# yjhuangcd/FI-ODE

Hardware: AMD Instinct MI355X
Metric: CIFAR-10 train-step images/sec (B=128, h_sample=256) at 1/2/4/8 MI355X (higher is better)
Workload: dtype f32; 1 GPU; hipGraph replay: BASELINE configs[1]: train step of README.md:27 at epoch 20 with train_ode (rk4, step_size 0.1, t_max=1: 10 steps / 40 train-mode f-evals, backprop through the stages; loss_ode portion 0.2) + the Lyapunov loss (B=128, h_sample_size=256 -> 204 uniform + 52 correct-cone rows/image), KWLarge-Cayley backbone + Adam; global_batch=128, h_sample_size=256, rows_per_rank=32768, parallelism=dp1

## Files before the change

### fi-ode_amd/csrc/odetrain.hip

```cpp
#include <type_traits>
#include "common.h"
#include "tile.h"
#include "tile16.h"
#include "tile4.h"
#include "wgrad.h"
#include "dopri5.h"
#include "../../include/fiode.h"

namespace {
using namespace fiode_tile;
using namespace fiode_t16;
using namespace fiode_t4;
using namespace fiode_dp;


constexpr int OT_XRING = 4;
constexpr int FIODE_OT_KW_PRE = 256;

struct OTArgs {
  int prio;
  int B, E, niters;
  int nslots;
  int kw_lazy;
  int kw_pre;
// ... 317 lines not shown
    store_row10(a.ftw + r * C, ft);
    store_row10(a.nomw + r * C, nominal);
    store_row10(a.loww + r * C, lower);
    store_row10(a.vw + r * C, k);
    a.muw[r] = mu;
  }
  if (blockIdx.x == 0 && threadIdx.x == 0) a.stats[2] = K;
#ifdef OT_PROFILE
  if (blockIdx.x == 0 && threadIdx.x == 0 && e < 96) a.prof[16 + e] = (unsigned long long)K;
#endif
  if (threadIdx.x == 0) sh.Kprev = K;
  if (end_barrier) __syncthreads();
  OT_MARK(4);
}

__global__ __launch_bounds__(256) void k_ot_fwd4(OTArgs a) {
  fiode_wave_prio(a.prio & 1);
  extern __shared__ __attribute__((aligned(16))) float smem[];
  OtShared4& sh = *reinterpret_cast<OtShared4*>(smem);
  if (threadIdx.x == 0) {
    sh.Kprev = a.d.max_iter - 1;
    sh.dead = 0;
  }
  const int lane = threadIdx.x & 63, j = lane & 3;
  const int p = __builtin_amdgcn_readfirstlane(threadIdx.x >> 6);
  const int b = blockIdx.x * TR4 + j;
  const bool valid = b < a.B;
  const int bb = valid ? b : a.B - 1;
  T4W w;
  load_t4w(a.Q1, a.Q2, a.Q3, a.b2, a.b3, p, lane, w);
  for (int t = threadIdx.x; t < TR4 * M; t += blockDim.x) {
    const int rb = blockIdx.x * TR4 + t / M, i = t % M;
    if (rb < a.B) {
      float s = 0.f;
#pragma unroll
      for (int c = 0; c < FIODE_X; ++c) s = __fmaf_rn(a.Qx[i * FIODE_X + c], a.x_feat[(size_t)rb * FIODE_X + c], s);
      a.u[(size_t)rb * M + i] = (s + a.bx[i]) + a.b1[i];
    }
  }
  __syncthreads();
  const f32x4 uacc = *reinterpret_cast<const f32x4*>(a.u + (size_t)bb * M + 32 * p + 4 * ((lane >> 2) & 7));
  const uint32_t* kwp = a.kw;
  auto fetch = [&](int e, uint32_t& w1, uint32_t& w2) {
    if (a.dropout_mode == FIODE_DROPOUT_OFF) {
      w1 = w2 = 0xFFFFFFFFu;
      return;
    }
    w1 = kwp[(((size_t)e * 2 + 0) * a.B + bb) * 4 + p];
    w2 = kwp[(((size_t)e * 2 + 1) * a.B + bb) * 4 + p];
  };
  uint32_t kc1, kc2, kn1 = 0u, kn2 = 0u;
  fetch(0, kc1, kc2);
  float y[C], k1[C], k2[C], k3[C], k4[C], hin[C];
  load_row10(a.h0 + (size_t)bb * C, y);
  const float third = 1.0f / 3.0f;
  const int eN = 4 * (a.niters - 1);
  for (int it = 0; it + 1 < a.niters; ++it) {
    float ta, dt;
    step_times(a, it, ta, dt);
    const int e0 = 4 * it;
#define OT4_STAGE(E_, H_, K_)                                                            \
    {                                                                                    \
      if ((E_) + 1 < eN) fetch((E_) + 1, kn1, kn2);                                      \
      ot_eval4(a, w, sh, (E_), p, b, valid, lane, j, uacc, kc1, kc2, H_, K_, false);    \
      kc1 = kn1;                                                                         \
      kc2 = kn2;                                                                         \
    }
    OT4_STAGE(e0, y, k1)
// ... 10 lines not shown
#pragma unroll
    for (int i = 0; i < C; ++i) {
      const float dy = (((k1[i] + 3.0f * (k2[i] + k3[i])) + k4[i]) * dt) * 0.125f;
      y[i] = y[i] + dy;
    }
  }
  if (sh.dead) {
#pragma unroll
    for (int i = 0; i < C; ++i) y[i] = __builtin_nanf("");
  }
  if (p == 0 && valid && lane < TR4) store_row10(a.y_out + (size_t)b * C, y);
  if (blockIdx.x == 0 && threadIdx.x == 0) {
    a.stats[0] = 4 * (a.niters - 1);
    a.stats[1] = a.niters - 1;
  }
}

struct OtBwdShared {
  float gpart[2][4][64][4];
  float gax[8][64][4];
};

struct VjpIn {
  float h[C], ft[C], v[C], mu;
  f32x4 a2[2];
  f32x4 a1[2];
};

__device__ __forceinline__ void load_vjp_in(const OTArgs& a, int p, int e, int b, bool valid, int q, VjpIn& in) {
  const int bb = valid ? b : a.B - 1;
// ... 340 lines not shown
  if (blk4 < 4) *reinterpret_cast<f32x4*>(&sh.gpart[buf][p][lane][0]) = f32x4{gh[0], gh[1], gh[2], gh[3]};
  OT_MARK(13);
  __syncthreads();
  OT_MARK(14);
#pragma unroll
  for (int i = 0; i < C; ++i) {
    const int ln = 4 * (i >> 2) + j, rg = i & 3;
    const float ghm = ((sh.gpart[buf][0][ln][rg] + sh.gpart[buf][1][ln][rg]) + sh.gpart[buf][2][ln][rg]) +
                      sh.gpart[buf][3][ln][rg];
    gy_out[i] = ghm + ghb[i];
  }
  OT_MARK(15);
}

template <bool SN>
__global__ __launch_bounds__(256) void k_ot_bwd4(OTArgs a) {
  fiode_wave_prio(a.prio & 2);
  extern __shared__ __attribute__((aligned(16))) float smem[];
  OtBwdShared4& sh = *reinterpret_cast<OtBwdShared4*>(smem);
  const int lane = threadIdx.x & 63, j = lane & 3;
  const int p = __builtin_amdgcn_readfirstlane(threadIdx.x >> 6);
  VjpW4 wv;
  {
    const int bq = lane >> 2, i = lane & 3;
    const int u = 32 * p + 4 * (bq & 7) + i;
#pragma unroll
    for (int s = 0; s < 5; ++s) wv.q3t[s] = a.Q3[(s + 5 * (bq >> 3)) * M + u];
#pragma unroll
    for (int s = 0; s < 64; ++s) wv.q2t[s] = a.Q2[(size_t)(s + 64 * (bq >> 3)) * M + u];
    const int c = 4 * (bq & 3) + i;
#pragma unroll
    for (int s = 0; s < 8; ++s) wv.q1t[s] = c < C ? a.Q1[(32 * p + 8 * (bq >> 2) + s) * C + c] : 0.f;
  }
  const int b = blockIdx.x * TR4 + j;
  const bool valid = b < a.B;
  float gy[C];
  if (valid) load_row10(a.g_y + (size_t)b * C, gy);
  else
#pragma unroll
    for (int i = 0; i < C; ++i) gy[i] = 0.f;
  const float third = 1.0f / 3.0f;
  int buf = 0;
  VjpIn4 cur, nxt;
  VjpRow crw;
  load_vjp_in4(a, p, a.E - 1, b, valid, lane, cur);
#define OT_VJP4(E_, G_)                                                                 \
  load_vjp_in4(a, p, (E_) - 1, b, valid, lane, nxt);                                    \
  vjp_row_math<SN>(a, cur, crw);                                                        \
  ot_vjp4<SN>(a, wv, sh, buf, p, (E_), b, valid, lane, j, cur, crw, G_, gY);          \
  cur = nxt;                                                                            \
  buf ^= 1;
  for (int it = a.niters - 2; it >= 0; --it) {
    float ta, dt;
    step_times(a, it, ta, dt);
    const float c8 = dt * 0.125f, c38 = 3.0f * c8;
// ... 23 lines not shown
      const float d = dt * gY[i];
      gk2[i] += d;
      gk1[i] -= d * third;
    }
    OT_VJP4(e0 + 1, gk2)
#pragma unroll
    for (int i = 0; i < C; ++i) {
      acc[i] += gY[i];
      gk1[i] += (dt * gY[i]) * third;
    }
    OT_VJP4(e0, gk1)
#pragma unroll
    for (int i = 0; i < C; ++i) gy[i] = acc[i] + gY[i];
  }
#undef OT_VJP4
}

constexpr int OT_XV = 4;
enum { ALOG_T = 0, ALOG_DT, ALOG_RATIO, ALOG_ACCEPT, ALOG_FIDX, ALOG_E0, ALOG_W = 8 };
enum { META_D0 = 0, META_D1, META_D2, META_H0, META_H1, META_CLAMP0, META_CLAMP1, META_DT0, META_R2, META_N = 16 };

template <int N>
__device__ __forceinline__ double dpp_row_shr(double x) {
  const long long u = __double_as_longlong(x);
  const int lo = __builtin_amdgcn_update_dpp(0, (int)(u & 0xFFFFFFFF), 0x110 + N, 0xf, 0xf, true);
  const int hi = __builtin_amdgcn_update_dpp(0, (int)(u >> 32), 0x110 + N, 0xf, 0xf, true);
  return __longlong_as_double(((long long)(unsigned)hi << 32) | (unsigned)lo);
}
__device__ __forceinline__ double readlane_d(double x, int l) {
  const long long u = __double_as_longlong(x);
// ... 1016 lines not shown
  FIODE_HIP_CHECK(hipGetLastError());
  if (a.method == FIODE_ODE_DOPRI5) {
    if ((a.B + TR4 - 1) / TR4 <= FIODE_OT4_MAX_TILES)
      hipLaunchKernelGGL(k_odp_fwd<true>, dim3((a.B + TR4 - 1) / TR4), dim3(256), sizeof(OdpShared<true>), st, a);
    else
      hipLaunchKernelGGL(k_odp_fwd<false>, dim3(ntiles), dim3(256), sizeof(OdpShared<false>), st, a);
  } else if ((a.B + TR4 - 1) / TR4 <= FIODE_OT4_MAX_TILES) {
    hipLaunchKernelGGL(k_ot_fwd4, dim3((a.B + TR4 - 1) / TR4), dim3(256), sizeof(OtShared4), st, a);
  } else {
    hipLaunchKernelGGL(k_ot_fwd, dim3(ntiles), dim3(256), sizeof(OtShared), st, a);
  }
  FIODE_HIP_CHECK(hipGetLastError());
  return FIODE_OK;
}

namespace {
__global__ __launch_bounds__(M) void k_ot_gx(int E, const int32_t* __restrict__ e_used, const float* __restrict__ gz1,
                                             const float* __restrict__ Qx, const float* __restrict__ add,
                                             const float* __restrict__ scale, float* __restrict__ gx) {
  __shared__ float gu[M];
  const int b = blockIdx.x, m = threadIdx.x;
  const float* p = gz1 + (size_t)b * E * M + m;
  const int En = e_used ? min(E, e_used[0]) : E;
  float s = 0.f;
#pragma unroll 8
  for (int e = 0; e < En; ++e) s += p[(size_t)e * M];
  gu[m] = s;
  __syncthreads();
  if (m < FIODE_X) {
    float d = 0.f;
// ... 60 lines not shown
  hipStream_t st = static_cast<hipStream_t>(stream);
  FIODE_HIP_CHECK(launch_sweep(a, st));
  const OtLayout L = ot_layout(a.B, a.E, a.A);
  fiode_internal::WgradIO io{};
  io.B = a.B; io.S = a.E; io.x_feat = x_feat; io.Qx = w->Qx; io.h = a.hs; io.a1 = a.a1; io.a2 = a.a2;
  io.s_used = a.method == FIODE_ODE_DOPRI5 ? a.imeta : nullptr;
  io.gz2 = a.gz2; io.gz1 = a.gz1; io.gft = a.gft;
  io.workspace = static_cast<char*>(workspace) + L.wg;
  io.grads = *grads;
  return fiode_internal::launch_wgrad(st, io);
}

namespace {
__global__ __launch_bounds__(256) void k_ode_nll(int B, const float* __restrict__ y_hat, const int64_t* __restrict__ y,
                                                 float* __restrict__ loss, float* __restrict__ gunit,
                                                 const float* __restrict__ lyap, float p, float* __restrict__ mix) {
  __shared__ float red[256];
  const int tid = threadIdx.x;
  float s = 0.f;
  for (int b = tid; b < B; b += 256) {
    const int64_t l = y[b];
    const bool ok = l >= 0 && l < C;
    const float v = ok ? y_hat[(size_t)b * C + l] : __builtin_nanf("");
    s = s + (-logf(v));
    const float g0 = -1.0f / ((float)B * v);
    const float g = mix ? g0 * p : g0;
#pragma unroll
    for (int c = 0; c < C; ++c) gunit[(size_t)b * C + c] = (c == l) ? g : 0.f;
  }
  red[tid] = s;
  __syncthreads();
#pragma unroll
  for (int o = 128; o > 0; o >>= 1) {
// ... 13 lines not shown
  if (batch <= 0 || !y_hat || !labels || !loss || !g_unit) return FIODE_EINVAL;
  hipLaunchKernelGGL(k_ode_nll, dim3(1), dim3(256), 0, static_cast<hipStream_t>(stream), batch, y_hat, labels, loss,
                     g_unit, nullptr, 0.0f, nullptr);
  FIODE_HIP_CHECK(hipGetLastError());
  return FIODE_OK;
}

extern "C" int fiode_ode_loss_mix(void* stream, int32_t batch, const float* y_hat, const int64_t* labels,
                                  const float* lyap_loss, float portion, float* loss_ode, float* total, float* g_unit) {
  if (batch <= 0 || !y_hat || !labels || !lyap_loss || !loss_ode || !total || !g_unit) return FIODE_EINVAL;
  hipLaunchKernelGGL(k_ode_nll, dim3(1), dim3(256), 0, static_cast<hipStream_t>(stream), batch, y_hat, labels,
                     loss_ode, g_unit, lyap_loss, portion, total);
  FIODE_HIP_CHECK(hipGetLastError());
  return FIODE_OK;
}
```

### fi-ode_amd/fiode_amd/_lib.py

```python
from __future__ import annotations

import ctypes as ct
import os
import pathlib

_HERE = pathlib.Path(__file__).resolve().parent
LIB_PATH = pathlib.Path(os.environ.get("FIODE_LIB", _HERE / "libfiode.so"))

FIODE_SAMPLER_GIVEN, FIODE_SAMPLER_COMPOSITE, FIODE_SAMPLER_DECISION_BOUNDARY, FIODE_SAMPLER_TRAJECTORY = 0, 1, 2, 3
FIODE_DROPOUT_OFF, FIODE_DROPOUT_GIVEN, FIODE_DROPOUT_PHILOX = 0, 1, 2
FIODE_ACT_RELU, FIODE_ACT_GROUPSORT = 0, 1

class FiodeLibraryError(RuntimeError):
    pass


class FiodeError(RuntimeError):
    pass


_fp = ct.POINTER(ct.c_float)
_vp = ct.c_void_p


# ... 140 lines not shown
                                         ct.c_int32]),
        "fiode_odetrain_evals": (ct.c_int32, [ct.POINTER(OdeTrainConfig)]),
        "fiode_odetrain_saved_offsets": (ct.c_int, [ct.POINTER(OdeTrainConfig), _vp]),
        "fiode_odetrain_workspace_bytes": (ct.c_size_t, [ct.POINTER(OdeTrainConfig)]),
        "fiode_odetrain_forward": (ct.c_int, [_vp, ct.POINTER(OdeTrainConfig), ct.POINTER(DynConfig),
                                              ct.POINTER(DynWeights), _vp, _vp, _vp, _vp, _vp, _vp, _vp, ct.c_size_t]),
        "fiode_odetrain_backward": (ct.c_int, [_vp, ct.POINTER(OdeTrainConfig), ct.POINTER(DynConfig),
                                               ct.POINTER(DynWeights), _vp, _vp, ct.POINTER(LyapGrads), _vp, _vp,
                                               ct.c_size_t]),
        "fiode_odetrain_backward_x": (ct.c_int, [_vp, ct.POINTER(OdeTrainConfig), ct.POINTER(DynConfig),
                                                 ct.POINTER(DynWeights), _vp, _vp, _vp, _vp, _vp, _vp, _vp,
                                                 ct.c_size_t]),
        "fiode_odetrain_backward_weights": (ct.c_int, [_vp, ct.POINTER(OdeTrainConfig), ct.POINTER(DynConfig),
                                                       ct.POINTER(DynWeights), _vp, ct.POINTER(LyapGrads), _vp,
                                                       ct.c_size_t]),
        "fiode_groupsort_forward": (ct.c_int, [_vp, ct.c_int64, ct.c_int64, ct.c_int64, _vp, _vp]),
        "fiode_groupsort_backward": (ct.c_int, [_vp, ct.c_int64, ct.c_int64, ct.c_int64, _vp, _vp, _vp]),
        "fiode_head_out": (ct.c_int, [_vp, ct.c_int32, ct.c_int32, ct.c_int32, _vp, _vp, _vp, _vp]),
        "fiode_head_out_backward_gs": (ct.c_int, [_vp, ct.c_int32, ct.c_int32, ct.c_int32, _vp, _vp, _vp, _vp]),
        "fiode_batched_inverse": (ct.c_int, [_vp, ct.c_int32, ct.c_int32, ct.c_int32, _vp, ct.c_int64, _vp,
                                             ct.c_int64]),
        "fiode_block_inverse_workspace_bytes": (ct.c_size_t, [ct.c_int32]),
        "fiode_block_inverse": (ct.c_int, [_vp, ct.c_int32, _vp, _vp, _vp, ct.c_size_t]),
        "fiode_block_inverse_batched": (ct.c_int, [_vp, ct.c_int32, ct.c_int32, _vp, _vp, _vp, ct.c_size_t]),
        "fiode_block_inverse_cond": (ct.c_int, [_vp, ct.c_int32, ct.c_int32, _vp, _vp, _vp, ct.c_size_t, _vp]),
        "fiode_normalize_hwcb": (ct.c_int, [_vp, ct.c_int32, ct.c_int32, ct.c_int32, ct.c_int32, _vp, _vp, _vp, _vp]),
        "fiode_ode_nll": (ct.c_int, [_vp, ct.c_int32, _vp, _vp, _vp, _vp]),
        "fiode_ode_loss_mix": (ct.c_int, [_vp, ct.c_int32, _vp, _vp, _vp, ct.c_float, _vp, _vp, _vp]),
        "fiode_small_cayley_forward": (ct.c_int, [_vp, ct.c_int32, ct.c_int32, ct.c_int32, _vp, _vp, _vp, _vp, _vp]),
        "fiode_small_cayley_backward": (ct.c_int, [_vp, ct.c_int32, ct.c_int32, ct.c_int32, _vp, _vp, _vp, _vp, _vp,
                                                   _vp, _vp]),
        "fiode_dense_cayley_prep": (ct.c_int, [_vp, ct.POINTER(DenseConfig), _vp, _vp, _vp, _vp, _vp]),
        "fiode_dense_norm_workspace_bytes": (ct.c_size_t, [ct.POINTER(DenseConfig)]),
        "fiode_dense_norm_partials": (ct.c_int, [_vp, ct.POINTER(DenseConfig), _vp, _vp, ct.c_size_t]),
        "fiode_dense_cayley_prep_normed": (ct.c_int, [_vp, ct.POINTER(DenseConfig), _vp, _vp, _vp, _vp, _vp, _vp]),
        "fiode_dense_norm_partials_clear": (ct.c_int, [_vp, ct.POINTER(DenseConfig), _vp, _vp, ct.c_size_t, _vp,
                                                       ct.c_size_t, ct.c_size_t]),
        "fiode_dense_inverse_flag_bytes": (ct.c_size_t, [ct.c_int32]),
        "fiode_dense_cayley_inverse": (ct.c_int, [_vp, ct.POINTER(DenseConfig), _vp, _vp, _vp, _vp, _vp, _vp, _vp,
                                                  _vp, ct.c_size_t]),
        "fiode_dense_cayley_finish": (ct.c_int, [_vp, ct.POINTER(DenseConfig), _vp, _vp, _vp, _vp, _vp]),
        "fiode_dense_cayley_ginv": (ct.c_int, [_vp, ct.POINTER(DenseConfig), _vp, _vp, _vp, _vp, _vp]),
        "fiode_dense_cayley_h": (ct.c_int, [_vp, ct.POINTER(DenseConfig), _vp, _vp, _vp]),
# ... 58 lines not shown
```

### fi-ode_amd/fiode_amd/graph_step.py

```python
from __future__ import annotations

import os
from typing import Optional

import torch

from .streams import StepStreams, distinct, new_stream, run_on

CAPTURE_PRIORITY = 0
CAPTURE_WS_SLOTS = 24


MIN_HW_QUEUES = 4


def _check_runtime_queues() -> None:
    q = os.environ.get("GPU_MAX_HW_QUEUES")
    if q is not None and q.strip().isdigit() and int(q) < MIN_HW_QUEUES:
        raise RuntimeError(f"GraphTrainStep: GPU_MAX_HW_QUEUES={q} < {MIN_HW_QUEUES}: this HIP runtime's graph "
                           "executor segfaults replaying a multi-branch graph with fewer hardware queues "
                           "(DESIGN.md section 6); unset it or use >= 4")


class GraphTrainStep:
    def __init__(self, module, optimizer, x: torch.Tensor, y: torch.Tensor, *, reducer=None, world: int = 1,
                 warmup: int = 3, act: str = "relu", check_every: int = 200, maps_ahead: bool = True,
                 comm: Optional[str] = None, bucket_bytes: int = 4 << 20, force_comm: bool = False,
                 guard: bool = True, placement_trials: int = 1, warm_capture: bool = True):
        _check_runtime_queues()
        dev = x.device
        if dev.type != "cuda":
            raise ValueError("GraphTrainStep needs ROCm device tensors")
        module.require_trainable_dynamics("GraphTrainStep")
        self.module, self.opt, self.reducer, self.world, self.act = module, optimizer, reducer, world, act
        self.check_every, self.n_replays = int(check_every), 0
        self.piped, self.early = [], False
        self.force_comm = bool(force_comm)
        multi = reducer is not None and (world > 1 or self.force_comm)
        if comm is None:
            import torch.distributed as dist
            comm = "graph" if (multi and dist.is_initialized() and dist.get_backend() == "nccl") else "eager"
        if comm not in ("graph", "eager"):
            raise ValueError(f"comm must be 'graph' or 'eager', got {comm!r}")
        self.comm = comm if multi else "none"
# ... 227 lines not shown
                            st[k] = old[k]
                        continue
                    if old is not None and k in old and torch.is_tensor(old[k]):
                        v.copy_(old[k])
                    else:
                        v.zero_()
            self.module.rng_counter.copy_(counter)

    def _fwd_bwd(self, bucket_plan: bool = True):
        m = self.module
        for p in self.params:
            p.grad = None
        overlap = self.comm == "graph" and bucket_plan
        if overlap:
            self.reducer.arm(self.world, m.streams.comm, force=self.force_comm)
        loss = m.compute_loss(self.static_x, self.static_y, self.static_x.shape[0], self.act)
        self._arm_guard(loss)
        loss.backward(self._unit_grad(loss))
        if overlap:
            self.reducer.finish()
        elif self.comm != "none":
            self.reducer.gather()
        m.rng_counter.add_(1)
        return loss

    def _unit_grad(self, loss):
        from .lyapunov import UNIT_GRAD
        u = getattr(self, "_unit", None)
        if u is None or u.device != loss.device or u.dtype != loss.dtype:
            if torch.cuda.is_current_stream_capturing():
                raise RuntimeError("GraphTrainStep: the unit gradient seed must exist before the capture")
# ... 60 lines not shown
```

### fi-ode_amd/fiode_amd/lyapunov.py

```python
from __future__ import annotations

import contextlib
from typing import Dict, Optional

import numpy as np
import torch
import torch.nn as nn
import torch.nn.functional as F

from . import _lib as L
from . import ops
from .dynamics import OrthoClassDynProjectSimplexLips
from .models import IVP, DefaultOutputFun
from .odeint import make_solver_params
from .optim import FiodeAdam, FiodeAdamW
from .sampling import CompositeSampler, CompositeSamplerScheduler, TrajectorySampler
from .streams import StepStreams, current, prefetch, run_on, take


@contextlib.contextmanager
def no_param_grad(module: nn.Module):
    flags = [(p, p.requires_grad) for p in module.parameters()]
    modes = [(m, m.training) for m in module.modules()]
    try:
# ... 126 lines not shown
        fn = ctx.box.pop("weights")
        ctx.box = None
        return (None,) + tuple(fn())


class LyapODELossFn(torch.autograd.Function):

    @staticmethod
    def forward(ctx, x_feat, x_ode, Q1, b1, Qx, bx, Q2, b2, Q3, b3, h0, y, plan: dict, oplan: dict, p: float,
                ode_stream, box=None, tok=None):
        w = {"Q1": Q1, "b1": b1, "Qx": Qx, "bx": bx, "Q2": Q2, "b2": b2, "Q3": Q3, "b3": b3}
        w = {k: v.detach().contiguous() for k, v in w.items()}
        xf = x_feat.detach().float().contiguous()
        xo = xf if x_ode is None else x_ode.detach().float().contiguous()

        def solve():
            return ops.odetrain_forward(xo, h0.detach().float().contiguous(), w, oplan["dyn"], oplan["cfg"],
                                        masks=oplan.get("masks"), offset_dev=oplan.get("offset_dev"))
        pre = prefetch(ode_stream, solve) if ode_stream is not None else None
        res = None if pre is not None else solve()
        sc, grads, dbg = ops.lyap_step(
            xf, y, w, plan["dyn"], sample_size=plan["S"], n_uniform=plan["S1"],
            sampler=plan["sampler"], dropout_mode=plan["dropout_mode"], kappa=plan["kappa"], seed=plan["seed"],
            offset=plan["offset"], h=plan.get("h"), masks=plan.get("masks"), debug=plan.get("debug", False),
            out=plan.get("out"), offset_dev=plan.get("offset_dev"), kappa_dev=plan.get("kappa_dev"))
        plan["scalars"] = sc
        plan["debug_out"] = dbg
        ctx.lyap = [grads[k] for k in ("x_feat", "Q1", "b1", "Qx", "bx", "Q2", "b2", "Q3", "b3")]
        ctx.lyap_unit = torch._foreach_mul(ctx.lyap, 1.0 - float(p))
        if pre is not None:
            res = take(pre)
        y_hat, stats, ws = res
        oplan["stats"] = stats
        oplan["status_word"] = ops.odetrain_status_word(ws, oplan["cfg"])
        B = y_hat.shape[0]
        total = torch.empty((), dtype=torch.float32, device=y_hat.device)
        loss_ode = torch.empty((), dtype=torch.float32, device=y_hat.device)
        gunit = torch.empty_like(y_hat)
        L.check(L.lib().fiode_ode_loss_mix(ops._stream(y_hat.device), B, y_hat.data_ptr(), y.contiguous().data_ptr(),
                                           sc.data_ptr(), float(p), loss_ode.data_ptr(), total.data_ptr(),
                                           gunit.data_ptr()), "fiode_ode_loss_mix")
        plan["loss_ode"] = loss_ode
        plan["y_hat"] = y_hat
        ctx.ode = (gunit, xo, w, oplan, ws)
        ctx.p = float(p)
        ctx.split = x_ode is not None
        ctx.box = box
        return total

    @staticmethod
    def backward(ctx, go):
        gunit, xo, w, oplan, ws = ctx.ode
        ctx.ode = None
        unit = getattr(go, UNIT_GRAD, False)
        g_y = gunit if unit else gunit * go
        box, ctx.box = ctx.box, None
        if box is not None:
            lyap = ctx.lyap_unit if unit else torch._foreach_mul(ctx.lyap, go * (1.0 - ctx.p))
            ctx.lyap = ctx.lyap_unit = None
            if ctx.split:
                gxo = ops.odetrain_backward_x(g_y, xo, w, oplan["dyn"], oplan["cfg"], ws)
                gx = lyap[0]
            else:
                gx = ops.odetrain_backward_x(g_y, xo, w, oplan["dyn"], oplan["cfg"], ws, gx_add=lyap[0],
                                             gx_add_scale=_one(g_y.device))
                gxo = None

            def weights():
                side = torch.cuda.current_stream(xo.device)
                for t in [xo, ws] + list(w.values()) + list(lyap[1:]):
                    t.record_stream(side)
                gr = ops.odetrain_backward_weights(xo, w, oplan["dyn"], oplan["cfg"], ws)
                ode = [gr[k] for k in ("Q1", "b1", "Qx", "bx", "Q2", "b2", "Q3", "b3")]
                torch._foreach_add_(ode, lyap[1:])
                return ode
            box["weights"] = weights
            tg = go if go.dim() == 0 else go.reshape(())
# ... 75 lines not shown
        self.fix_backbone = fix_backbone
        self.decay_epochs, self.betas = list(decay_epochs), (beta1, beta2)
        self.scheduler_name, self.max_epochs, self.warmup = scheduler_name, max_epochs, warmup
        self.simplex, self.act, self.eps, self.norm = simplex, act, eps, norm
        self.val_adv = bool(val_adv)
        self.val_adv_generator: Optional[torch.Generator] = None
        self.epoch_off_scale = epoch_off_scale
        self.current_epoch = 0
        self.global_step = 0
        self.seed = seed
        self._rng_offset = 0
        self.rng_counter: Optional[torch.Tensor] = None
        self.parallel_cayley = True
        self.lyap_after_ode = False
        self.ode_reuse_features = True
        self.fused_ode_loss = True
        self.streams = StepStreams()
        self._prefetch_late_at = 2
        self.logged: Dict[str, float] = {}
        self._out = None

    @property
    def dyn_fun(self):
        return self.model.dyn_fun

    @property
    def init_coordinates(self):
        return self.model.init_coordinates

    @property
# ... 269 lines not shown
        key = (B, h0_0.device, h0_0.data_ptr(), h0_0._version)
        c = getattr(self, "_h0_cache", None)
        if c is not None and c[0] == key:
            return c[1]
        h0 = h0_0[None].expand(B, -1).float().contiguous()
        if not (h0.is_cuda and torch.cuda.is_current_stream_capturing()):
            self._h0_cache = (key, h0)
        return h0

    def _lyap_ode_loss(self, x, static_state, w, y, plan):
        x_ode = None
        if not self.ode_reuse_features:
            x_ode, _ = self.init_coordinates(x, self.dyn_fun)
        h0 = self._h0(static_state.shape[0])
        oplan = self.ode_plan(static_state.shape[0])
        self.last_ode_plan = oplan
        stream = self._ode_stream(static_state.device) if self.parallel_cayley else None
        p = min(0.98, (self.current_epoch - self.train_ode_epoch) / 50.0)
        keys = ("Q1", "b1", "Qx", "bx", "Q2", "b2", "Q3", "b3")
        if DYN_WGRAD_SIDE and static_state.is_cuda and torch.is_grad_enabled():
            box = {}
            tok = run_on(self.streams.get("wtap", static_state.device),
                         lambda: _DynWeightTapFn.apply(box, *[w[k] for k in keys]))
            wd = [w[k].detach() for k in keys]
            total = LyapODELossFn.apply(static_state, x_ode, *wd, h0, y, plan, oplan, p, stream, box, tok)
        else:
            total = LyapODELossFn.apply(static_state, x_ode, *[w[k] for k in keys], h0, y, plan, oplan, p, stream)
        sc = plan["scalars"]
        self.log("kappa", plan["kappa_dev"] if plan.get("kappa_dev") is not None else plan["kappa"])
        self.log("effective_batch_size", sc[1])
# ... 21 lines not shown
```

### fi-ode_amd/fiode_amd/ops.py

```python
from __future__ import annotations

import ctypes as ct
from dataclasses import dataclass
from typing import Dict, Optional

import torch

from . import _lib as L

C, M, X = 10, 128, 10
WEIGHT_KEYS = ("Q1", "b1", "Qx", "bx", "Q2", "b2", "Q3", "b3")
WEIGHT_SHAPES = {"Q1": (M, C), "b1": (M,), "Qx": (M, X), "bx": (M,), "Q2": (M, M), "b2": (M,),
                 "Q3": (C, M), "b3": (C,)}


@dataclass
class DynCfg:
    alpha_1: float = 100.0
    alpha_2: float = 20.0
    sigma_1: float = 0.02
    scale_nominal: bool = True
    dropout: float = 0.5
    qp_max_iter: int = 30
    qp_tol: float = 1e-4
# ... 422 lines not shown
        masks = _need(masks, "masks", (E, 2, B, M), torch.uint8, dev)
    if offset_dev is not None:
        offset_dev = _need(offset_dev, "offset_dev", (1,), torch.int64, dev)
    lib = L.lib()
    ws = torch.empty(lib.fiode_odetrain_workspace_bytes(ct.byref(cfg)), dtype=torch.uint8, device=dev)
    ws_w, cw = _weights_c(weights, dev)
    y = torch.empty((B, C), dtype=torch.float32, device=dev)
    stats = torch.empty(8, dtype=torch.int32, device=dev)
    dc = dyn.to_c()
    rc = lib.fiode_odetrain_forward(_stream(dev), ct.byref(cfg), ct.byref(dc), ct.byref(cw), x_feat.data_ptr(),
                                    h0.data_ptr(), _ptr(masks), _ptr(offset_dev), y.data_ptr(), stats.data_ptr(),
                                    ws.data_ptr(), ws.numel())
    L.check(rc, "fiode_odetrain_forward")
    del ws_w
    return y, stats, ws


def odetrain_saved(ws: torch.Tensor, cfg: L.OdeTrainConfig) -> Dict[str, torch.Tensor]:
    B, E = int(cfg.batch), odetrain_evals(cfg)
    off = (ct.c_int64 * L.FIODE_ODETRAIN_NSAVED)()
    L.check(L.lib().fiode_odetrain_saved_offsets(ct.byref(cfg), ct.cast(off, ct.c_void_p)),
            "fiode_odetrain_saved_offsets")
    f = lambda i, n: ws[off[i]:off[i] + 4 * n].view(torch.float32)
    R = B * E
    out = dict(h=f(0, R * C).view(B, E, C), ftilde=f(1, R * C).view(B, E, C), v=f(2, R * C).view(B, E, C),
               mu=f(3, R).view(B, E), nominal=f(4, R * C).view(B, E, C), a1=f(5, R * M).view(B, E, M),
               a2=f(6, R * M).view(B, E, M), gft=f(7, R * C).view(B, E, C), lower=f(8, R * C).view(B, E, C),
               status=ws[off[12]:off[12] + 4].view(torch.int32),
               keep_words=ws[off[13]:off[13] + E * 2 * B * 16].view(torch.int32).view(E, 2, B, 4))
    if cfg.method == L.FIODE_ODE_DOPRI5:
# ... 460 lines not shown
```

### include/fiode.h

```cpp
#ifndef FIODE_H_
#define FIODE_H_

#include <stddef.h>
#include <stdint.h>

#ifdef __cplusplus
extern "C" {
#endif

#define FIODE_ABI_VERSION 5

#if defined(__GNUC__)
#define FIODE_API __attribute__((visibility("default")))
#else
#define FIODE_API
#endif

enum {
  FIODE_OK = 0,
  FIODE_EINVAL = 1,
  FIODE_ESHAPE = 2,
  FIODE_EWORKSPACE = 3,
  FIODE_EHIP = 100
};
// ... 158 lines not shown
                            float* g_unit);
FIODE_API int fiode_ode_loss_mix(void* stream, int32_t batch, const float* y_hat, const int64_t* labels,
                                 const float* lyap_loss, float portion, float* loss_ode, float* total, float* g_unit);
FIODE_API int fiode_odetrain_backward(void* stream, const fiode_odetrain_config* cfg, const fiode_dyn_config* dyn,
                                      const fiode_dyn_weights* w, const float* x_feat, const float* g_y,
                                      fiode_lyap_grads* grads, float* dbg_gft, void* workspace,
                                      size_t workspace_bytes);
FIODE_API int fiode_odetrain_backward_x(void* stream, const fiode_odetrain_config* cfg, const fiode_dyn_config* dyn,
                                        const fiode_dyn_weights* w, const float* x_feat, const float* g_y, float* gx,
                                        const float* gx_add, const float* gx_add_scale, float* dbg_gft,
                                        void* workspace, size_t workspace_bytes);
FIODE_API int fiode_odetrain_backward_weights(void* stream, const fiode_odetrain_config* cfg,
                                              const fiode_dyn_config* dyn, const fiode_dyn_weights* w,
                                              const float* x_feat, fiode_lyap_grads* grads, void* workspace,
                                              size_t workspace_bytes);

typedef struct fiode_certify_config {
  int32_t n_classes;
  int32_t T;
  int32_t batches;
  int32_t label;
  float eps;
  float min_std;
} fiode_certify_config;

FIODE_API int64_t fiode_certify_grid_rows(int32_t n, int32_t T);
FIODE_API int fiode_certify_grid(void* stream, int32_t n, int32_t T, uint8_t* grid);
FIODE_API size_t fiode_certify_workspace_bytes(int64_t G, int32_t batches);
FIODE_API int fiode_certify(void* stream, const fiode_certify_config* cfg, const fiode_dyn_config* dyn,
                            const fiode_dyn_weights* w, const float* x_feat, const uint8_t* grid, int64_t G,
// ... 158 lines not shown
```

Before: 105,400 images/s.

## Fuse ODE forward solve, unit-gradient backward, and gx reduction into one kernel

Adds a k_ot_solve4 kernel that runs the RK4 forward, computes the NLL unit gradient on-device from the labels, runs the VJP backward, and reduces gz1 through Qx into gx_ode, all in one launch on the ODE prefetch stream. The loss-mix kernel now also combines gx_ode with the Lyapunov gx, and the later backward_x launch is skipped when the unit gradient applies. The aim is to move the ODE backward off the critical backward path and overlap it with the Lyapunov work, while removing launches. In exchange the fused path assumes the incoming gradient is the unit gradient, and it applies only to RK4 with ReLU; graph capture turns it on by default.

```diff
diff --git a/fi-ode_amd/csrc/odetrain.hip b/fi-ode_amd/csrc/odetrain.hip
--- a/fi-ode_amd/csrc/odetrain.hip
+++ b/fi-ode_amd/csrc/odetrain.hip
@@ -355,18 +355,12 @@
   OT_MARK(4);
 }
 
-__global__ __launch_bounds__(256) void k_ot_fwd4(OTArgs a) {
-  fiode_wave_prio(a.prio & 1);
-  extern __shared__ __attribute__((aligned(16))) float smem[];
-  OtShared4& sh = *reinterpret_cast<OtShared4*>(smem);
+__device__ __forceinline__ void ot_fwd4_body(const OTArgs& a, OtShared4& sh, int lane, int j, int p, int b, bool valid,
+                                             float (&y)[C]) {
   if (threadIdx.x == 0) {
     sh.Kprev = a.d.max_iter - 1;
     sh.dead = 0;
   }
-  const int lane = threadIdx.x & 63, j = lane & 3;
-  const int p = __builtin_amdgcn_readfirstlane(threadIdx.x >> 6);
-  const int b = blockIdx.x * TR4 + j;
-  const bool valid = b < a.B;
   const int bb = valid ? b : a.B - 1;
   T4W w;
   load_t4w(a.Q1, a.Q2, a.Q3, a.b2, a.b3, p, lane, w);
@@ -392,7 +386,7 @@
   };
   uint32_t kc1, kc2, kn1 = 0u, kn2 = 0u;
   fetch(0, kc1, kc2);
-  float y[C], k1[C], k2[C], k3[C], k4[C], hin[C];
+  float k1[C], k2[C], k3[C], k4[C], hin[C];
   load_row10(a.h0 + (size_t)bb * C, y);
   const float third = 1.0f / 3.0f;
   const int eN = 4 * (a.niters - 1);
@@ -433,6 +427,17 @@
     a.stats[0] = 4 * (a.niters - 1);
     a.stats[1] = a.niters - 1;
   }
+}
+
+__global__ __launch_bounds__(256) void k_ot_fwd4(OTArgs a) {
+  fiode_wave_prio(a.prio & 1);
+  extern __shared__ __attribute__((aligned(16))) float smem[];
+  OtShared4& sh = *reinterpret_cast<OtShared4*>(smem);
+  const int lane = threadIdx.x & 63, j = lane & 3;
+  const int p = __builtin_amdgcn_readfirstlane(threadIdx.x >> 6);
+  const int b = blockIdx.x * TR4 + j;
+  float y[C];
+  ot_fwd4_body(a, sh, lane, j, p, b, b < a.B, y);
 }
 
 struct OtBwdShared {
@@ -803,12 +808,8 @@
 }
 
 template <bool SN>
-__global__ __launch_bounds__(256) void k_ot_bwd4(OTArgs a) {
-  fiode_wave_prio(a.prio & 2);
-  extern __shared__ __attribute__((aligned(16))) float smem[];
-  OtBwdShared4& sh = *reinterpret_cast<OtBwdShared4*>(smem);
-  const int lane = threadIdx.x & 63, j = lane & 3;
-  const int p = __builtin_amdgcn_readfirstlane(threadIdx.x >> 6);
+__device__ __forceinline__ void ot_bwd4_body(const OTArgs& a, OtBwdShared4& sh, int lane, int j, int p, int b,
+                                             bool valid, float (&gy)[C]) {
   VjpW4 wv;
   {
     const int bq = lane >> 2, i = lane & 3;
@@ -821,13 +822,6 @@
 #pragma unroll
     for (int s = 0; s < 8; ++s) wv.q1t[s] = c < C ? a.Q1[(32 * p + 8 * (bq >> 2) + s) * C + c] : 0.f;
   }
-  const int b = blockIdx.x * TR4 + j;
-  const bool valid = b < a.B;
-  float gy[C];
-  if (valid) load_row10(a.g_y + (size_t)b * C, gy);
-  else
-#pragma unroll
-    for (int i = 0; i < C; ++i) gy[i] = 0.f;
   const float third = 1.0f / 3.0f;
   int buf = 0;
   VjpIn4 cur, nxt;
@@ -881,6 +875,81 @@
     for (int i = 0; i < C; ++i) gy[i] = acc[i] + gY[i];
   }
 #undef OT_VJP4
+}
+
+template <bool SN>
+__global__ __launch_bounds__(256) void k_ot_bwd4(OTArgs a) {
+  fiode_wave_prio(a.prio & 2);
+  extern __shared__ __attribute__((aligned(16))) float smem[];
+  OtBwdShared4& sh = *reinterpret_cast<OtBwdShared4*>(smem);
+  const int lane = threadIdx.x & 63, j = lane & 3;
+  const int p = __builtin_amdgcn_readfirstlane(threadIdx.x >> 6);
+  const int b = blockIdx.x * TR4 + j;
+  const bool valid = b < a.B;
+  float gy[C];
+  if (valid) load_row10(a.g_y + (size_t)b * C, gy);
+  else
+#pragma unroll
+    for (int i = 0; i < C; ++i) gy[i] = 0.f;
+  ot_bwd4_body<SN>(a, sh, lane, j, p, b, valid, gy);
+}
+
+union OtSolveShared4 {
+  OtShared4 fwd;
+  OtBwdShared4 bwd;
+  float gu[TR4][M];
+};
+
+template <bool SN>
+__global__ __launch_bounds__(256) void k_ot_solve4(OTArgs a, const int64_t* __restrict__ labels, float portion,
+                                                   float* __restrict__ gx_ode) {
+  extern __shared__ __attribute__((aligned(16))) float smem[];
+  OtSolveShared4& sh = *reinterpret_cast<OtSolveShared4*>(smem);
+  const int lane = threadIdx.x & 63, j = lane & 3;
+  const int p = __builtin_amdgcn_readfirstlane(threadIdx.x >> 6);
+  const int b = blockIdx.x * TR4 + j;
+  const bool valid = b < a.B;
+  fiode_wave_prio(a.prio & 1);
+  float y[C];
+  ot_fwd4_body(a, sh.fwd, lane, j, p, b, valid, y);
+  float gy[C];
+  {
+    const int64_t l = valid ? labels[b] : 0;
+    float v = __builtin_nanf("");
+#pragma unroll
+    for (int c = 0; c < C; ++c) v = (l == c) ? y[c] : v;
+    const float g0 = -1.0f / ((float)a.B * v);
+    const float g = g0 * portion;
+#pragma unroll
+    for (int c = 0; c < C; ++c) gy[c] = (valid && c == l) ? g : 0.f;
+  }
+  __syncthreads();
+  fiode_wave_prio(a.prio & 2);
+  ot_bwd4_body<SN>(a, sh.bwd, lane, j, p, b, valid, gy);
+  __syncthreads();
+  {
+    const int m = threadIdx.x & (M - 1);
+    for (int rr = threadIdx.x / M; rr < TR4; rr += 256 / M) {
+      const int rb = blockIdx.x * TR4 + rr;
+      if (rb >= a.B) continue;
+      const float* g = a.gz1 + (size_t)rb * a.E * M + m;
+      float s = 0.f;
+#pragma unroll 8
+      for (int e = 0; e < a.E; ++e) s += g[(size_t)e * M];
+      sh.gu[rr][m] = s;
+    }
+  }
+  __syncthreads();
+  if (threadIdx.x < TR4 * 16) {
+    const int rr = threadIdx.x >> 4, x = threadIdx.x & 15;
+    const int rb = blockIdx.x * TR4 + rr;
+    if (x < FIODE_X && rb < a.B) {
+      float d = 0.f;
+#pragma unroll 16
+      for (int i = 0; i < M; ++i) d = __fmaf_rn(sh.gu[rr][i], a.Qx[i * FIODE_X + x], d);
+      gx_ode[(size_t)rb * FIODE_X + x] = d;
+    }
+  }
 }
 
 constexpr int OT_XV = 4;
@@ -1927,6 +1996,41 @@
   return FIODE_OK;
 }
 
+extern "C" int fiode_odetrain_solve_unit(void* stream, const fiode_odetrain_config* cfg, const fiode_dyn_config* dyn,
+                                         const fiode_dyn_weights* w, const float* x_feat, const float* h0,
+                                         const uint8_t* masks, const uint64_t* offset_dev, const int64_t* labels,
+                                         float portion, float* y_out, int32_t* stats, float* gx_ode, void* workspace,
+                                         size_t workspace_bytes, int32_t activation) {
+  if (!labels || !gx_ode || !h0 || !y_out || !stats) return FIODE_EINVAL;
+  if (activation != FIODE_ACT_RELU && activation != FIODE_ACT_GROUPSORT) return FIODE_EINVAL;
+  OTArgs a{};
+  a.prio = (int)g_fiode_prio_mask;
+  int rc = fill_args(a, cfg, dyn, w, x_feat, workspace, workspace_bytes);
+  if (rc && rc != FIODE_EWORKSPACE) return rc;
+  if (activation != FIODE_ACT_RELU || cfg->method != FIODE_ODE_RK4 ||
+      (cfg->batch + TR4 - 1) / TR4 > FIODE_OT4_MAX_TILES)
+    return FIODE_ESHAPE;
+  if (rc) return rc;
+  if (a.dropout_mode == FIODE_DROPOUT_GIVEN && !masks) return FIODE_EINVAL;
+  a.h0 = h0; a.masks = masks; a.offset_dev = offset_dev; a.y_out = y_out; a.stats = stats;
+  a.drop_block = fiode_internal::debug_drop_publish();
+  hipStream_t st = static_cast<hipStream_t>(stream);
+  const OtLayout L = ot_layout(a.B, a.E, a.A);
+  a.nslots = (int)((L.kw - L.xs) / 8);
+  a.kw_lazy = 0;
+  a.kw_pre = a.E;
+  const int nthreads = std::max(a.nslots, a.kw_pre * a.B);
+  hipLaunchKernelGGL(k_ot_masks, dim3((nthreads + 255) / 256), dim3(256), 0, st, a);
+  FIODE_HIP_CHECK(hipGetLastError());
+  const dim3 grid((a.B + TR4 - 1) / TR4);
+  if (a.d.scale_nominal)
+    hipLaunchKernelGGL(k_ot_solve4<true>, grid, dim3(256), sizeof(OtSolveShared4), st, a, labels, portion, gx_ode);
+  else
+    hipLaunchKernelGGL(k_ot_solve4<false>, grid, dim3(256), sizeof(OtSolveShared4), st, a, labels, portion, gx_ode);
+  FIODE_HIP_CHECK(hipGetLastError());
+  return FIODE_OK;
+}
+
 namespace {
 __global__ __launch_bounds__(M) void k_ot_gx(int E, const int32_t* __restrict__ e_used, const float* __restrict__ gz1,
                                              const float* __restrict__ Qx, const float* __restrict__ add,
@@ -2017,9 +2121,17 @@
 namespace {
 __global__ __launch_bounds__(256) void k_ode_nll(int B, const float* __restrict__ y_hat, const int64_t* __restrict__ y,
                                                  float* __restrict__ loss, float* __restrict__ gunit,
-                                                 const float* __restrict__ lyap, float p, float* __restrict__ mix) {
+                                                 const float* __restrict__ lyap, float p, float* __restrict__ mix,
+                                                 const float* __restrict__ gx_ode = nullptr,
+                                                 const float* __restrict__ gx_add = nullptr,
+                                                 const float* __restrict__ gx_scale = nullptr,
+                                                 float* __restrict__ gx = nullptr) {
   __shared__ float red[256];
   const int tid = threadIdx.x;
+  if (gx) {
+    const float sc = gx_scale[0];
+    for (int t = tid; t < B * FIODE_X; t += 256) gx[t] = gx_ode[t] + gx_add[t] * sc;
+  }
   float s = 0.f;
   for (int b = tid; b < B; b += 256) {
     const int64_t l = y[b];
@@ -2063,3 +2175,16 @@
   FIODE_HIP_CHECK(hipGetLastError());
   return FIODE_OK;
 }
+
+extern "C" int fiode_ode_loss_mix_gx(void* stream, int32_t batch, const float* y_hat, const int64_t* labels,
+                                     const float* lyap_loss, float portion, float* loss_ode, float* total,
+                                     float* g_unit, const float* gx_ode, const float* gx_add,
+                                     const float* gx_add_scale, float* gx) {
+  if (batch <= 0 || !y_hat || !labels || !lyap_loss || !loss_ode || !total || !g_unit || !gx_ode || !gx_add ||
+      !gx_add_scale || !gx)
+    return FIODE_EINVAL;
+  hipLaunchKernelGGL(k_ode_nll, dim3(1), dim3(256), 0, static_cast<hipStream_t>(stream), batch, y_hat, labels,
+                     loss_ode, g_unit, lyap_loss, portion, total, gx_ode, gx_add, gx_add_scale, gx);
+  FIODE_HIP_CHECK(hipGetLastError());
+  return FIODE_OK;
+}
diff --git a/fi-ode_amd/fiode_amd/_lib.py b/fi-ode_amd/fiode_amd/_lib.py
--- a/fi-ode_amd/fiode_amd/_lib.py
+++ b/fi-ode_amd/fiode_amd/_lib.py
@@ -178,6 +178,9 @@
         "fiode_odetrain_backward_weights": (ct.c_int, [_vp, ct.POINTER(OdeTrainConfig), ct.POINTER(DynConfig),
                                                        ct.POINTER(DynWeights), _vp, ct.POINTER(LyapGrads), _vp,
                                                        ct.c_size_t]),
+        "fiode_odetrain_solve_unit": (ct.c_int, [_vp, ct.POINTER(OdeTrainConfig), ct.POINTER(DynConfig),
+                                                 ct.POINTER(DynWeights), _vp, _vp, _vp, _vp, _vp, ct.c_float, _vp,
+                                                 _vp, _vp, _vp, ct.c_size_t, ct.c_int32]),
         "fiode_groupsort_forward": (ct.c_int, [_vp, ct.c_int64, ct.c_int64, ct.c_int64, _vp, _vp]),
         "fiode_groupsort_backward": (ct.c_int, [_vp, ct.c_int64, ct.c_int64, ct.c_int64, _vp, _vp, _vp]),
         "fiode_head_out": (ct.c_int, [_vp, ct.c_int32, ct.c_int32, ct.c_int32, _vp, _vp, _vp, _vp]),
@@ -191,6 +194,8 @@
         "fiode_normalize_hwcb": (ct.c_int, [_vp, ct.c_int32, ct.c_int32, ct.c_int32, ct.c_int32, _vp, _vp, _vp, _vp]),
         "fiode_ode_nll": (ct.c_int, [_vp, ct.c_int32, _vp, _vp, _vp, _vp]),
         "fiode_ode_loss_mix": (ct.c_int, [_vp, ct.c_int32, _vp, _vp, _vp, ct.c_float, _vp, _vp, _vp]),
+        "fiode_ode_loss_mix_gx": (ct.c_int, [_vp, ct.c_int32, _vp, _vp, _vp, ct.c_float, _vp, _vp, _vp, _vp, _vp,
+                                             _vp, _vp]),
         "fiode_small_cayley_forward": (ct.c_int, [_vp, ct.c_int32, ct.c_int32, ct.c_int32, _vp, _vp, _vp, _vp, _vp]),
         "fiode_small_cayley_backward": (ct.c_int, [_vp, ct.c_int32, ct.c_int32, ct.c_int32, _vp, _vp, _vp, _vp, _vp,
                                                    _vp, _vp]),
diff --git a/fi-ode_amd/fiode_amd/graph_step.py b/fi-ode_amd/fiode_amd/graph_step.py
--- a/fi-ode_amd/fiode_amd/graph_step.py
+++ b/fi-ode_amd/fiode_amd/graph_step.py
@@ -22,12 +22,17 @@
                            "(DESIGN.md section 6); unset it or use >= 4")
 
 
+FUSED_SOLVE = True
+
+
 class GraphTrainStep:
     def __init__(self, module, optimizer, x: torch.Tensor, y: torch.Tensor, *, reducer=None, world: int = 1,
                  warmup: int = 3, act: str = "relu", check_every: int = 200, maps_ahead: bool = True,
                  comm: Optional[str] = None, bucket_bytes: int = 4 << 20, force_comm: bool = False,
-                 guard: bool = True, placement_trials: int = 1, warm_capture: bool = True):
+                 guard: bool = True, placement_trials: int = 1, warm_capture: bool = True,
+                 fused_solve: bool = FUSED_SOLVE):
         _check_runtime_queues()
+        self.fused_solve = bool(fused_solve)
         dev = x.device
         if dev.type != "cuda":
             raise ValueError("GraphTrainStep needs ROCm device tensors")
@@ -285,7 +290,11 @@
         overlap = self.comm == "graph" and bucket_plan
         if overlap:
             self.reducer.arm(self.world, m.streams.comm, force=self.force_comm)
-        loss = m.compute_loss(self.static_x, self.static_y, self.static_x.shape[0], self.act)
+        fused, m.ode_fused_unit = getattr(m, "ode_fused_unit", False), self.fused_solve
+        try:
+            loss = m.compute_loss(self.static_x, self.static_y, self.static_x.shape[0], self.act)
+        finally:
+            m.ode_fused_unit = fused
         self._arm_guard(loss)
         loss.backward(self._unit_grad(loss))
         if overlap:
diff --git a/fi-ode_amd/fiode_amd/lyapunov.py b/fi-ode_amd/fiode_amd/lyapunov.py
--- a/fi-ode_amd/fiode_amd/lyapunov.py
+++ b/fi-ode_amd/fiode_amd/lyapunov.py
@@ -164,7 +164,14 @@
         xf = x_feat.detach().float().contiguous()
         xo = xf if x_ode is None else x_ode.detach().float().contiguous()
 
+        fused = bool(oplan.get("fused_unit")) and x_ode is None and box is not None and \
+            ops.odetrain_solve_unit_served(oplan["dyn"], oplan["cfg"])
+
         def solve():
+            if fused:
+                return ops.odetrain_solve_unit(xo, h0.detach().float().contiguous(), w, oplan["dyn"], oplan["cfg"],
+                                               y.contiguous(), float(p), masks=oplan.get("masks"),
+                                               offset_dev=oplan.get("offset_dev"))
             return ops.odetrain_forward(xo, h0.detach().float().contiguous(), w, oplan["dyn"], oplan["cfg"],
                                         masks=oplan.get("masks"), offset_dev=oplan.get("offset_dev"))
         pre = prefetch(ode_stream, solve) if ode_stream is not None else None
@@ -180,16 +187,22 @@
         ctx.lyap_unit = torch._foreach_mul(ctx.lyap, 1.0 - float(p))
         if pre is not None:
             res = take(pre)
-        y_hat, stats, ws = res
+        y_hat, stats, ws = res[:3]
         oplan["stats"] = stats
         oplan["status_word"] = ops.odetrain_status_word(ws, oplan["cfg"])
         B = y_hat.shape[0]
-        total = torch.empty((), dtype=torch.float32, device=y_hat.device)
-        loss_ode = torch.empty((), dtype=torch.float32, device=y_hat.device)
-        gunit = torch.empty_like(y_hat)
-        L.check(L.lib().fiode_ode_loss_mix(ops._stream(y_hat.device), B, y_hat.data_ptr(), y.contiguous().data_ptr(),
-                                           sc.data_ptr(), float(p), loss_ode.data_ptr(), total.data_ptr(),
-                                           gunit.data_ptr()), "fiode_ode_loss_mix")
+        ctx.gx_unit = None
+        if fused:
+            loss_ode, total, gunit, ctx.gx_unit = ops.ode_loss_mix_gx(y_hat, y.contiguous(), sc, float(p), res[3],
+                                                                      ctx.lyap_unit[0], _one(y_hat.device))
+        else:
+            total = torch.empty((), dtype=torch.float32, device=y_hat.device)
+            loss_ode = torch.empty((), dtype=torch.float32, device=y_hat.device)
+            gunit = torch.empty_like(y_hat)
+            L.check(L.lib().fiode_ode_loss_mix(ops._stream(y_hat.device), B, y_hat.data_ptr(),
+                                               y.contiguous().data_ptr(), sc.data_ptr(), float(p),
+                                               loss_ode.data_ptr(), total.data_ptr(), gunit.data_ptr()),
+                    "fiode_ode_loss_mix")
         plan["loss_ode"] = loss_ode
         plan["y_hat"] = y_hat
         ctx.ode = (gunit, xo, w, oplan, ws)
@@ -208,9 +221,12 @@
         if box is not None:
             lyap = ctx.lyap_unit if unit else torch._foreach_mul(ctx.lyap, go * (1.0 - ctx.p))
             ctx.lyap = ctx.lyap_unit = None
+            gx_unit, ctx.gx_unit = ctx.gx_unit, None
             if ctx.split:
                 gxo = ops.odetrain_backward_x(g_y, xo, w, oplan["dyn"], oplan["cfg"], ws)
                 gx = lyap[0]
+            elif unit and gx_unit is not None:
+                gx, gxo = gx_unit, None
             else:
                 gx = ops.odetrain_backward_x(g_y, xo, w, oplan["dyn"], oplan["cfg"], ws, gx_add=lyap[0],
                                              gx_add_scale=_one(g_y.device))
@@ -316,6 +332,7 @@
         self.parallel_cayley = True
         self.lyap_after_ode = False
         self.ode_reuse_features = True
+        self.ode_fused_unit = False
         self.fused_ode_loss = True
         self.streams = StepStreams()
         self._prefetch_late_at = 2
@@ -615,6 +632,7 @@
             x_ode, _ = self.init_coordinates(x, self.dyn_fun)
         h0 = self._h0(static_state.shape[0])
         oplan = self.ode_plan(static_state.shape[0])
+        oplan["fused_unit"] = bool(self.ode_fused_unit)
         self.last_ode_plan = oplan
         stream = self._ode_stream(static_state.device) if self.parallel_cayley else None
         p = min(0.98, (self.current_epoch - self.train_ode_epoch) / 50.0)
diff --git a/fi-ode_amd/fiode_amd/ops.py b/fi-ode_amd/fiode_amd/ops.py
--- a/fi-ode_amd/fiode_amd/ops.py
+++ b/fi-ode_amd/fiode_amd/ops.py
@@ -460,6 +460,64 @@
     L.check(rc, "fiode_odetrain_forward")
     del ws_w
     return y, stats, ws
+
+
+ODETRAIN_OT4_MAX_ROWS = 1024
+
+
+def odetrain_solve_unit_served(dyn: DynCfg, cfg: L.OdeTrainConfig) -> bool:
+    return dyn.activation == "ReLU" and cfg.method == L.FIODE_ODE_RK4 and int(cfg.batch) <= ODETRAIN_OT4_MAX_ROWS
+
+
+def odetrain_solve_unit(x_feat: torch.Tensor, h0: torch.Tensor, weights: Dict[str, torch.Tensor], dyn: DynCfg,
+                        cfg: L.OdeTrainConfig, labels: torch.Tensor, portion: float,
+                        masks: Optional[torch.Tensor] = None, offset_dev: Optional[torch.Tensor] = None):
+    dev = h0.device
+    B = int(cfg.batch)
+    h0 = _need(h0, "h0", (B, C), torch.float32, dev)
+    x_feat = _need(x_feat, "x_feat", (B, X), torch.float32, dev)
+    labels = _need(labels, "labels", (B,), torch.int64, dev)
+    E = odetrain_evals(cfg)
+    if cfg.dropout_mode == L.FIODE_DROPOUT_GIVEN:
+        if masks is None:
+            raise ValueError("dropout GIVEN needs masks [E,2,B,M]")
+        masks = _need(masks, "masks", (E, 2, B, M), torch.uint8, dev)
+    if offset_dev is not None:
+        offset_dev = _need(offset_dev, "offset_dev", (1,), torch.int64, dev)
+    lib = L.lib()
+    ws = torch.empty(lib.fiode_odetrain_workspace_bytes(ct.byref(cfg)), dtype=torch.uint8, device=dev)
+    ws_w, cw = _weights_c(weights, dev)
+    y = torch.empty((B, C), dtype=torch.float32, device=dev)
+    stats = torch.empty(8, dtype=torch.int32, device=dev)
+    gx_ode = torch.empty((B, X), dtype=torch.float32, device=dev)
+    dc = dyn.to_c()
+    rc = lib.fiode_odetrain_solve_unit(_stream(dev), ct.byref(cfg), ct.byref(dc), ct.byref(cw), x_feat.data_ptr(),
+                                       h0.data_ptr(), _ptr(masks), _ptr(offset_dev), labels.data_ptr(),
+                                       float(portion), y.data_ptr(), stats.data_ptr(), gx_ode.data_ptr(),
+                                       ws.data_ptr(), ws.numel(), _act(dyn))
+    L.check(rc, "fiode_odetrain_solve_unit")
+    del ws_w
+    return y, stats, ws, gx_ode
+
+
+def ode_loss_mix_gx(y_hat: torch.Tensor, labels: torch.Tensor, lyap_loss: torch.Tensor, portion: float,
+                    gx_ode: torch.Tensor, gx_add: torch.Tensor, gx_add_scale: torch.Tensor):
+    dev = y_hat.device
+    B = int(y_hat.shape[0])
+    y_hat = _need(y_hat, "y_hat", (B, C), torch.float32, dev)
+    labels = _need(labels, "labels", (B,), torch.int64, dev)
+    gx_ode = _need(gx_ode, "gx_ode", (B, X), torch.float32, dev)
+    gx_add = _need(gx_add, "gx_add", (B, X), torch.float32, dev)
+    gx_add_scale = _need(gx_add_scale.reshape(1), "gx_add_scale", (1,), torch.float32, dev)
+    total = torch.empty((), dtype=torch.float32, device=dev)
+    loss_ode = torch.empty((), dtype=torch.float32, device=dev)
+    gunit = torch.empty_like(y_hat)
+    gx = torch.empty((B, X), dtype=torch.float32, device=dev)
+    L.check(L.lib().fiode_ode_loss_mix_gx(_stream(dev), B, y_hat.data_ptr(), labels.data_ptr(), lyap_loss.data_ptr(),
+                                          float(portion), loss_ode.data_ptr(), total.data_ptr(), gunit.data_ptr(),
+                                          gx_ode.data_ptr(), gx_add.data_ptr(), gx_add_scale.data_ptr(),
+                                          gx.data_ptr()), "fiode_ode_loss_mix_gx")
+    return loss_ode, total, gunit, gx
 
 
 def odetrain_saved(ws: torch.Tensor, cfg: L.OdeTrainConfig) -> Dict[str, torch.Tensor]:
diff --git a/include/fiode.h b/include/fiode.h
--- a/include/fiode.h
+++ b/include/fiode.h
@@ -196,6 +196,15 @@
                                               const fiode_dyn_config* dyn, const fiode_dyn_weights* w,
                                               const float* x_feat, fiode_lyap_grads* grads, void* workspace,
                                               size_t workspace_bytes);
+FIODE_API int fiode_odetrain_solve_unit(void* stream, const fiode_odetrain_config* cfg, const fiode_dyn_config* dyn,
+                                        const fiode_dyn_weights* w, const float* x_feat, const float* h0,
+                                        const uint8_t* masks, const uint64_t* offset_dev, const int64_t* labels,
+                                        float portion, float* y_out, int32_t* stats, float* gx_ode,
+                                        void* workspace, size_t workspace_bytes, int32_t activation);
+FIODE_API int fiode_ode_loss_mix_gx(void* stream, int32_t batch, const float* y_hat, const int64_t* labels,
+                                    const float* lyap_loss, float portion, float* loss_ode, float* total,
+                                    float* g_unit, const float* gx_ode, const float* gx_add,
+                                    const float* gx_add_scale, float* gx);
 
 typedef struct fiode_certify_config {
   int32_t n_classes;
```

After: 107,300 images/s (median of 6 runs). 1.8% higher.
